# nv-tlabs/InfiniCube

Hardware: AMD Instinct MI355X
Metric: denoise steps/sec, 93-frame 480p Wan2.1 buffer-conditioned DiT loop (higher is better)
Workload: dtype bf16

## Files before the change

infinicube_amd/csrc/attention.hip:

```cpp
#include "icv_common.h"


int icv_attn1_dispatch(const void* q, int64_t ldq, const void* k, int64_t ldk, const void* v, int64_t ldv, void* o,
                       int64_t ldo, int64_t Sq, int64_t Skv, int64_t heads, float scale, void* stream);
int icv_attn2_dispatch(const void* q, int64_t ldq, const void* k, int64_t ldk, const void* v, int64_t ldv,
                       void* o, int64_t ldo, float* acc, int64_t ldacc, float* ml, int state_in,
                       int state_out, int64_t Sq, int64_t Skv, int64_t heads, float scale, int var,
                       hipStream_t st);

int icv_attn3_dispatch(const void* q, int64_t ldq, const void* k, int64_t ldk, const void* v, int64_t ldv,
                       void* o, int64_t ldo, float* acc, int64_t ldacc, float* ml, int state_in,
                       int state_out, int64_t Sq, int64_t Skv, int64_t heads, float scale, int var,
                       hipStream_t st);

int icv_attn9_dispatch(const void* q, int64_t ldq, const void* k, int64_t ldk, const void* v, int64_t ldv,
                       void* o, int64_t ldo, float* acc, int64_t ldacc, float* ml, int state_in,
                       int state_out, int64_t Sq, int64_t Skv, int64_t heads, float scale, int var,
                       hipStream_t st);
int icv_attn7p_single(const void* q, int64_t ldq, const void* k, int64_t ldk, const void* v, int64_t ldv, void* o, int64_t ldo, float* acc,
                      int64_t ldacc, float* ml, int state_in, int state_out, int64_t Sq, int64_t Skv, int64_t heads, float scale, hipStream_t st);
int icv_attn7q_single(const void* q, int64_t ldq, const void* k, int64_t ldk, const void* v, int64_t ldv, void* o, int64_t ldo, float* acc,
                      int64_t ldacc, float* ml, int state_in, int state_out, int64_t Sq, int64_t Skv, int64_t heads, float scale, int variant,
                      hipStream_t st);
int icv_attn7_dispatch(const void* q, int64_t ldq, const void* k, int64_t ldk, const void* v, int64_t ldv,
                       void* o, int64_t ldo, float* acc, int64_t ldacc, float* ml, int state_in,
                       int state_out, int64_t Sq, int64_t Skv, int64_t heads, float scale, int var,
                       hipStream_t st);
int icv_attn6_dispatch(const void* q, int64_t ldq, const void* k, int64_t ldk, const void* v, int64_t ldv,
                       void* o, int64_t ldo, float* acc, int64_t ldacc, float* ml, int state_in,
                       int state_out, int64_t Sq, int64_t Skv, int64_t heads, float scale, int var,
                       hipStream_t st);
int icv_attn5_dispatch(const void* q, int64_t ldq, const void* k, int64_t ldk, const void* v, int64_t ldv,
                       void* o, int64_t ldo, float* acc, int64_t ldacc, float* ml, int state_in,
                       int state_out, int64_t Sq, int64_t Skv, int64_t heads, float scale, int var,
                       hipStream_t st);
int icv_attn4_dispatch(const void* q, int64_t ldq, const void* k, int64_t ldk, const void* v, int64_t ldv,
                       void* o, int64_t ldo, float* acc, int64_t ldacc, float* ml, int state_in,
                       int state_out, int64_t Sq, int64_t Skv, int64_t heads, float scale, int var,
                       hipStream_t st);

constexpr int ATTN_KERNEL_DEFAULT = 7;
constexpr int ATTN7_VARIANT_DEFAULT = 132;
constexpr int ATTN7Q_DEFAULT = 0;
static int attn_route(const void* q, int64_t ldq, const void* k, int64_t ldk, const void* v, int64_t ldv, void* o,
                      int64_t ldo, float* acc, int64_t ldacc, float* ml, int state_in, int state_out, int64_t Sq,
                      int64_t Skv, int64_t heads, float scale, hipStream_t st) {
#define ATT_ARGS q, ldq, k, ldk, v, ldv, o, ldo, acc, ldacc, ml, state_in, state_out, Sq, Skv, heads, scale
  switch (icv_get_option_int("attn_kernel", ATTN_KERNEL_DEFAULT)) {
    case 7: {
      const int var7 = icv_get_option_int("attn7_variant", -1);
      int short_max = icv_get_option_int("attn7_short", -1);
      if (short_max < 0) short_max = 1024;
      if (var7 < 0 && Skv > short_max && !icv_get_option_int("attn7_plain", 0) && !icv_get_option_int("attn7_ablate", 0) && state_out != 2) {
#ifdef ICV_EXPERIMENTS
        const int q7 = icv_get_option_int("attn7q", ATTN7Q_DEFAULT);
        if (q7 > 0) {
          const int rc = icv_attn7q_single(ATT_ARGS, q7, st);
          if (rc >= 0) return rc;
        }
#endif
        return icv_attn7p_single(ATT_ARGS, st);
      }
      return icv_attn7_dispatch(ATT_ARGS, var7 < 0 ? ATTN7_VARIANT_DEFAULT : var7, st);
    }
#ifdef ICV_EXPERIMENTS
    case 9: return icv_attn9_dispatch(ATT_ARGS, icv_get_option_int("attn9_variant", 0), st);
    case 6: return icv_attn6_dispatch(ATT_ARGS, icv_get_option_int("attn6_variant", 5), st);
    case 5: return icv_attn5_dispatch(ATT_ARGS, 0, st);
    case 4: return icv_attn4_dispatch(ATT_ARGS, icv_get_option_int("attn4_variant", 4), st);
    case 3: return icv_attn3_dispatch(ATT_ARGS, icv_get_option_int("attn3_variant", 0), st);
#else
    case 9: case 6: case 5: case 4: case 3:
      icv_set_error("attn_kernel 3..6 and 9 are experiments: rebuild libicvideo with ICV_EXPERIMENTS=1");
      return 1;
#endif
    default: return icv_attn2_dispatch(ATT_ARGS, icv_get_option_int("attn2_variant", 12), st);
  }
#undef ATT_ARGS
}

extern "C" int icv_attention_fwd_chunk(const void* q, int64_t ldq, const void* k, int64_t ldk,
                                       const void* v, int64_t ldv, void* o, int64_t ldo, float* acc,
                                       int64_t ldacc, float* ml, int64_t Sq, int64_t Skv,
                                       int64_t heads, float scale, int first, int last, void* stream) {
  ICV_REQUIRE(q && k && v, "icv_attention_fwd_chunk: null pointer");
  ICV_REQUIRE(Sq > 0 && Skv > 0 && heads > 0, "icv_attention_fwd_chunk: empty problem");
  ICV_REQUIRE(ldq % 8 == 0 && ldk % 8 == 0 && ldv % 8 == 0, "icv_attention_fwd_chunk: leading dims must keep 16-byte row alignment");
  ICV_REQUIRE((first && last) || (acc && ml && ldacc % 4 == 0), "icv_attention_fwd_chunk: carried state buffers required unless first && last");
  ICV_REQUIRE(!last || (o && ldo % 4 == 0), "icv_attention_fwd_chunk: output required for the last chunk");
  return attn_route(q, ldq, k, ldk, v, ldv, o, ldo, acc, ldacc, ml, first ? 0 : 1, last ? 0 : 1, Sq, Skv, heads, scale, (hipStream_t)stream);
}

extern "C" int icv_attention_fwd(const void* q, int64_t ldq, const void* k, int64_t ldk,
                                 const void* v, int64_t ldv, void* o, int64_t ldo, int64_t Sq,
                                 int64_t Skv, int64_t heads, float scale, void* stream) {
  ICV_REQUIRE(q && k && v && o, "icv_attention_fwd: null pointer");
  ICV_REQUIRE(Sq > 0 && Skv > 0 && heads > 0, "icv_attention_fwd: empty problem (Sq=%lld Skv=%lld heads=%lld)", (long long)Sq, (long long)Skv, (long long)heads);
  ICV_REQUIRE(ldq % 8 == 0 && ldk % 8 == 0 && ldv % 8 == 0 && ldo % 4 == 0, "icv_attention_fwd: leading dims must keep 16-byte row alignment");
  if (icv_get_option_int("attn_kernel", ATTN_KERNEL_DEFAULT) != 1)
    return attn_route(q, ldq, k, ldk, v, ldv, o, ldo, nullptr, 0, nullptr, 0, 0, Sq, Skv, heads, scale, (hipStream_t)stream);
#ifdef ICV_EXPERIMENTS
  return icv_attn1_dispatch(q, ldq, k, ldk, v, ldv, o, ldo, Sq, Skv, heads, scale, stream);
#else
  icv_set_error("attn_kernel 1 is an experiment: rebuild libicvideo with ICV_EXPERIMENTS=1");
  return 1;
#endif
}

extern "C" int icv_attention_fwd_add(const void* q, int64_t ldq, const void* k, int64_t ldk,
                                     const void* v, int64_t ldv, void* o, int64_t ldo, int64_t Sq,
                                     int64_t Skv, int64_t heads, float scale, void* stream) {
  ICV_REQUIRE(q && k && v && o, "icv_attention_fwd_add: null pointer");
  ICV_REQUIRE(Sq > 0 && Skv > 0 && heads > 0, "icv_attention_fwd_add: empty problem (Sq=%lld Skv=%lld heads=%lld)", (long long)Sq, (long long)Skv, (long long)heads);
  ICV_REQUIRE(ldq % 8 == 0 && ldk % 8 == 0 && ldv % 8 == 0 && ldo % 4 == 0, "icv_attention_fwd_add: leading dims must keep 16-byte row alignment");
  return attn_route(q, ldq, k, ldk, v, ldv, o, ldo, nullptr, 0, nullptr, 0, 2, Sq, Skv, heads, scale, (hipStream_t)stream);
}

constexpr int ATTN_MFMA_DEFAULT = 16;
constexpr int ATTN_MFMA_SHORT_DEFAULT = 16;
int icv_attn_mfma(bool short_kv) {
  const int v = icv_get_option_int("attn_mfma", -1);
  if (v < 0) return short_kv ? ATTN_MFMA_SHORT_DEFAULT : ATTN_MFMA_DEFAULT;
  if (v == 16 || v == 32) return v;
  icv_set_error("attn_mfma = %d: the MFMA shape is 16 (16x16x32) or 32 (32x32x16); negative = the default", v);
  return -1;
}

constexpr int ATTN_TILE16_LEAN_DEFAULT = 1;
constexpr int ATTN_TILE16_LEAN_SHORT_DEFAULT = 1;
int icv_attn_tile16_lean(bool short_kv) {
  const int v = icv_get_option_int("attn_tile16_lean", -1);
  if (v < 0) return short_kv ? ATTN_TILE16_LEAN_SHORT_DEFAULT : ATTN_TILE16_LEAN_DEFAULT;
  if (v == 0 || v == 1) return v;
  icv_set_error("attn_tile16_lean = %d: 1 = the lean body of the 16x16x32 tile, 0 = the first body; negative = the default", v);
  return -1;
}

namespace {
unsigned long long* g_trace = nullptr;
int g_trace_cap = 0;
}
unsigned long long* icv_attention_trace_buffer(int* capacity) {
  *capacity = g_trace_cap;
  return g_trace;
}
extern "C" int icv_attention_trace(void* buf, int64_t capacity) {
  ICV_REQUIRE(capacity >= 0 && capacity < (1LL << 31), "icv_attention_trace: bad capacity");
  g_trace = (unsigned long long*)buf;
  g_trace_cap = buf ? (int)capacity : 0;
  return 0;
}
```

infinicube_amd/csrc/attn7p.hip:

```cpp
#include <type_traits>
#include "attn_common.h"

namespace att7p {

using attc::D;
using attc::NEG_BIG;
using attc::lds_read_tr16;
constexpr int KVB = 64;
constexpr int TILE_BYTES = KVB * D * 2;
constexpr int STAGE_BYTES = 2 * TILE_BYTES;
constexpr int NST = 4, NW = 8, NI = 16 / NW, QB = NW * 32;
constexpr int LDS_BYTES = NST * STAGE_BYTES + 64;
constexpr int MAX_PIECES = ICV_ATTN_MAX_PIECES;

struct Piece {
  const bf16_t* k;
  const bf16_t* v;
  int rows;
  int flag;
  unsigned value;
  int pad;
};

struct Params {
  attc::Params a;
  const unsigned* flags;
  unsigned* err;
  unsigned long long timeout_ticks;
  unsigned long long* ptrace;
  int n_pieces;
  Piece piece[MAX_PIECES];
  int fw_frames, fw_frame_rows, fw_window, fw_sink;
};

__device__ __forceinline__ void dma16(const void* gsrc, unsigned lds_dst) {
  unsigned keep;
  asm volatile(
      "s_mov_b32 %0, m0\n\t"
      "s_mov_b32 m0, %2\n\t"
      "s_nop 0\n\t"
      "global_load_lds_dwordx4 %1, off\n\t"
      "s_mov_b32 m0, %0"
      : "=&s"(keep)
      : "v"(gsrc), "s"(lds_dst)
      : "memory");
}

__device__ __forceinline__ void dma16s(const void* base, unsigned off, unsigned lds_dst) {
  unsigned keep;
  asm volatile(
      "s_mov_b32 %0, m0\n\t"
      "s_mov_b32 m0, %3\n\t"
      "s_nop 0\n\t"
      "global_load_lds_dwordx4 %1, %2\n\t"
      "s_mov_b32 m0, %0"
      : "=&s"(keep)
      : "v"(off), "s"(base), "s"(lds_dst)
      : "memory");
}

__device__ __forceinline__ unsigned load_flag_async(const unsigned* f) {
  unsigned v;
  asm volatile("global_load_dword %0, %1, off sc0 sc1" : "=v"(v) : "v"(f) : "memory");
  return v;
}

template <bool UNIT, bool FW, int MF, bool LEAN = false>
__global__ __launch_bounds__(NW * 64) __attribute__((amdgpu_waves_per_eu(2))) void attn7p_kernel(Params pp) {
  static_assert(MF == 16 || MF == 32, "MF: 16 (16x16x32 MFMAs) or 32 (32x32x16)");
  static_assert(MF == 16 || !LEAN, "the lean body is a body of the MF = 16 tile");
  const attc::Params& p = pp.a;
  const float p_lim = __builtin_amdgcn_exp2f(p.thr);
  extern __shared__ __attribute__((aligned(16))) char smem[];
  volatile unsigned* verdict = reinterpret_cast<volatile unsigned*>(smem + NST * STAGE_BYTES);
  const int tid = threadIdx.x;
  const int lane = tid & 63;
  const int wave = __builtin_amdgcn_readfirstlane(tid >> 6);
  const int hi = lane >> 5;
  const int l31 = lane & 31;

  int head, qb;
  attc::work_item(p, head, qb);
  int64_t q0 = (int64_t)qb * QB + wave * 32;
  int64_t q_end = 0;
  int fw_np = 1, fw_a0 = 0, fw_b0 = 0, fw_a1 = 0, fw_b1 = 0;
  if constexpr (FW) {
    const int T = pp.fw_frames, F = pp.fw_frame_rows, W = pp.fw_window, sink = pp.fw_sink;
    const int bpf = (F + QB - 1) / QB;
    const int f = qb / bpf;
    q0 = (int64_t)f * F + (qb - f * bpf) * QB + wave * 32;
    q_end = (int64_t)(f + 1) * F;
    const int lo = f - W > 0 ? f - W : 0;
    const int hi = f + W + 1 < T ? f + W + 1 : T;
    if (sink == 0) {
      fw_a0 = lo; fw_b0 = hi;
    } else if (lo <= sink) {
      fw_a0 = 0; fw_b0 = hi > sink ? hi : sink;
    } else {
      fw_np = 2;
      fw_a0 = 0; fw_b0 = sink;
      fw_a1 = lo; fw_b1 = hi;
    }
  }
  const unsigned long long t_start = p.trace ? __builtin_amdgcn_s_memrealtime() : 0ull;
  const bf16_t* qh = p.q + (int64_t)head * D;
  int64_t qr_c = q0 + l31;
  if constexpr (FW) qr_c = qr_c < q_end ? qr_c : q_end - 1;
  else qr_c = qr_c < p.Sq ? qr_c : p.Sq - 1;

  f32x16 ot[4];
  float m_run = NEG_BIG, l_run = 0.f;
  attc::Tile16 s16;
  int64_t qr16[2] = {0, 0};
  if constexpr (MF == 16) {
    const int64_t q_lim = FW ? q_end : p.Sq;
#pragma unroll
    for (int qb = 0; qb < 2; ++qb) {
      const int64_t r = q0 + qb * 16 + (lane & 15);
      qr16[qb] = r < q_lim ? r : q_lim - 1;
    }
    attc::tile16_init<UNIT>(p, qr16, head, lane >> 4, s16);
  } else {
    attc::load_state(p, qr_c, head, hi, ot, m_run, l_run);
  }
  float m_base = m_run < -1.0e29f ? 0.f : m_run;
  f32x16 cinit;
  const f32x16 zero16 = {0.f, 0.f, 0.f, 0.f, 0.f, 0.f, 0.f, 0.f, 0.f, 0.f, 0.f, 0.f, 0.f, 0.f, 0.f, 0.f};
#pragma unroll
  for (int r = 0; r < 16; ++r) cinit[r] = UNIT ? -m_base : 0.f;

  bf16x8 qf[8];
  if constexpr (MF == 16) attc::tile16_load_q(p, qr16, head, lane >> 4, s16);
  else {
    const bf16_t* qp = qh + qr_c * p.ldq + hi * 8;
#pragma unroll
    for (int ds = 0; ds < 8; ++ds) qf[ds] = *reinterpret_cast<const bf16x8*>(qp + ds * 16);
  }
  __builtin_amdgcn_s_waitcnt(0x0F70);

  const int pc = lane & 15;
  const unsigned lds_base = (unsigned)(uintptr_t)((__attribute__((address_space(3))) char*)smem);
  int dkey[NI], kcol[NI], vcol[NI];
  unsigned ko[NI], vo[NI];
#pragma unroll
  for (int j = 0; j < NI; ++j) {
    dkey[j] = (wave * NI + j) * 4 + (lane >> 4);
    kcol[j] = (pc ^ (dkey[j] & 15)) * 8;
    vcol[j] = MF == 16 ? attc::tile16_vcol(pc, dkey[j]) : (pc ^ ((dkey[j] & 3) << 2)) * 8;
    ko[j] = (unsigned)(((int64_t)dkey[j] * p.ldk + kcol[j]) * 2);
    vo[j] = (unsigned)(((int64_t)dkey[j] * p.ldv + vcol[j]) * 2);
  }

  const bf16_t* kh_d = nullptr;
  const bf16_t* vh_d = nullptr;
  int skv_d = 0, nt_d = 0;
#define P_ROWS(J_) (FW ? ((J_) ? fw_b1 - fw_a1 : fw_b0 - fw_a0) * pp.fw_frame_rows : __builtin_amdgcn_readfirstlane(pp.piece[FW ? 0 : (J_)].rows))
#define P_SET_DMA_PIECE(J_)                                              \
  {                                                                      \
    if constexpr (FW) {                                                  \
      const int64_t r0_ = (int64_t)((J_) ? fw_a1 : fw_a0) * pp.fw_frame_rows; \
      kh_d = p.k + r0_ * p.ldk + (int64_t)head * D;                      \
      vh_d = p.v + r0_ * p.ldv + (int64_t)head * D;                      \
      skv_d = P_ROWS(J_);                                                \
    } else {                                                             \
      const Piece& pc_ = pp.piece[(J_)];                                 \
      kh_d = pc_.k + (int64_t)head * D;                                  \
      vh_d = pc_.v + (int64_t)head * D;                                  \
      skv_d = __builtin_amdgcn_readfirstlane(pc_.rows);                  \
    }                                                                    \
    nt_d = (skv_d + KVB - 1) / KVB;                                      \
  }
#define P_DMA_TILE(T_, STG_)                                                                         \
  {                                                                                                  \
    const int tt_ = (T_) < nt_d ? (T_) : nt_d - 1;                                                   \
    const unsigned l0_ = lds_base + (unsigned)(((STG_) & (NST - 1)) * STAGE_BYTES + (wave * NI) * 1024); \
    if ((tt_ + 1) * KVB <= skv_d) {                                                                  \
      const bf16_t* kt_ = kh_d + (int64_t)tt_ * KVB * p.ldk;                                         \
      const bf16_t* vt_ = vh_d + (int64_t)tt_ * KVB * p.ldv;                                         \
      _Pragma("unroll") for (int j_ = 0; j_ < NI; ++j_) dma16s(kt_, ko[j_], l0_ + j_ * 1024);        \
      _Pragma("unroll") for (int j_ = 0; j_ < NI; ++j_) dma16s(vt_, vo[j_], l0_ + TILE_BYTES + j_ * 1024); \
    } else {                                                                                         \
      _Pragma("unroll") for (int j_ = 0; j_ < NI; ++j_) {                                            \
        int64_t r_ = (int64_t)tt_ * KVB + dkey[j_];                                                  \
        r_ = r_ < skv_d ? r_ : skv_d - 1;                                                            \
        dma16(kh_d + r_ * p.ldk + kcol[j_], l0_ + j_ * 1024);                                        \
        dma16(vh_d + r_ * p.ldv + vcol[j_], l0_ + TILE_BYTES + j_ * 1024);                           \
      }                                                                                              \
    }                                                                                                \
  }
#define P_BARRIER()                                           \
  do {                                                        \
    asm volatile("s_waitcnt lgkmcnt(0)" ::: "memory");        \
    __builtin_amdgcn_s_barrier();                             \
    asm volatile("" ::: "memory");                            \
    __builtin_amdgcn_sched_barrier(0);                        \
  } while (0)
#define P_WAIT_PIECE(J_)                                                                                          \
  if constexpr (!FW) {                                                                                            \
    const int fi_ = __builtin_amdgcn_readfirstlane(pp.piece[(J_)].flag);                                          \
    if (fi_ >= 0) {                                                                                               \
      if (tid == 0) {                                                                                             \
        const unsigned want_ = pp.piece[(J_)].value;                                                              \
        const unsigned long long t0_ = __builtin_amdgcn_s_memrealtime();                                          \
        while ((int)(__hip_atomic_load(pp.flags + fi_, __ATOMIC_RELAXED, __HIP_MEMORY_SCOPE_SYSTEM) - want_) < 0) { \
          __builtin_amdgcn_s_sleep(16);                                                                           \
              \
          if (pp.err && __hip_atomic_load(pp.err, __ATOMIC_RELAXED, __HIP_MEMORY_SCOPE_AGENT) != 0u) break;       \
          if (pp.timeout_ticks && __builtin_amdgcn_s_memrealtime() - t0_ > pp.timeout_ticks) {                    \
            if (pp.err) atomicCAS(pp.err, 0u, 0x80000000u | (unsigned)(J_));                                      \
            break;                                                                                                \
          }                                                                                                       \
        }                                                                                                         \
      }                                                                                                           \
      P_BARRIER();                                                                                                \
    }                                                                                                             \
  }

  const int k_row_off = l31 * 256;
  const int k_sw = l31 & 15;
  const int g = lane >> 4, t16 = lane & 15;
  const int v_key_lo = 4 * hi + (t16 >> 2);
  const int v_byte_lo = (g & 1) * 32 + (t16 & 3) * 8;
  const int v_sw = (t16 >> 2) << 6;

  attc::Tile16Addr la16;
  int la16_step = 2 * STAGE_BYTES;
  if constexpr (LEAN) {
    attc::tile16_lean_addr(lds_base, lane, la16);
    attc::tile16_lean_lim<UNIT>(s16, p_lim, la16);
  }
  auto tile = [&](const auto par, const int stg, const int key0, const int skv) __attribute__((always_inline)) {
    if constexpr (LEAN) {
      attc::tile16<UNIT, false, true, true, true, decltype(par)::value>(p, p_lim, nullptr, nullptr, key0, skv, lane, s16, &la16);
      return;
    }
    const char* ks = smem + (stg & (NST - 1)) * STAGE_BYTES;
    const char* vs = ks + TILE_BYTES;
    if constexpr (MF == 16) {
      attc::tile16<UNIT, false, true, true>(p, p_lim, ks, vs, key0, skv, lane, s16);
      return;
    }
    f32x16 st[2];
    const bool no_ref = UNIT && m_run < -1.0e29f;
#pragma unroll
    for (int ds = 0; ds < 8; ++ds)
#pragma unroll
      for (int kb = 0; kb < 2; ++kb) {
        const int c = ds * 2 + hi;
        const bf16x8 kf = *reinterpret_cast<const bf16x8*>(ks + kb * 8192 + k_row_off + ((c ^ k_sw) << 4));
        st[kb] = __builtin_amdgcn_mfma_f32_32x32x16_bf16(kf, qf[ds], ds == 0 ? (UNIT ? cinit : zero16) : st[kb], 0, 0, 0);
      }
    if (key0 + KVB > skv) {
#pragma unroll
      for (int kb = 0; kb < 2; ++kb)
#pragma unroll
        for (int r = 0; r < 16; ++r) {
          const int key = key0 + kb * 32 + (r & 3) + 8 * (r >> 2) + 4 * hi;
          if (key >= skv) st[kb][r] = NEG_BIG;
        }
    }
    float mb = -m_run * p.sc;
    float psum = 0.f;
    __builtin_amdgcn_s_setprio(1);
#pragma unroll
    for (int kb = 0; kb < 2; ++kb) {
      bf16x8 pf[2];
      float ps = 0.f;
#pragma unroll
      for (int r = 0; r < 16; ++r) {
        const float pv = UNIT ? __builtin_amdgcn_exp2f(st[kb][r]) : __builtin_amdgcn_exp2f(fmaf(st[kb][r], p.sc, mb));
        ps += pv;
        pf[r >> 3][r & 7] = (__bf16)pv;
      }
      if (__any(!(ps <= p_lim) || no_ref)) {
        float mloc = st[kb][0];
#pragma unroll
        for (int r = 1; r < 16; ++r) mloc = fmaxf(mloc, st[kb][r]);
        mloc = fmaxf(mloc, __shfl_xor(mloc, 32, 64));
        if (UNIT) mloc += m_base;
        const float m_new = fmaxf(m_run, mloc);
        const float alpha = __builtin_amdgcn_exp2f((m_run - m_new) * p.sc);
        m_run = m_new;
        l_run = (l_run + psum) * alpha;
        psum = 0.f;
#pragma unroll
        for (int i = 0; i < 4; ++i)
#pragma unroll
          for (int r = 0; r < 16; ++r) ot[i][r] *= alpha;
        mb = -m_run * p.sc;
        if (UNIT) {
          const float dm = m_new - m_base;
          m_base = m_new;
#pragma unroll
          for (int j = 0; j < 2; ++j)
            if (j >= kb) {
#pragma unroll
              for (int r = 0; r < 16; ++r) st[j][r] -= dm;
            }
#pragma unroll
          for (int r = 0; r < 16; ++r) cinit[r] = -m_new;
        }
        ps = 0.f;
#pragma unroll
        for (int r = 0; r < 16; ++r) {
          const float pv = UNIT ? __builtin_amdgcn_exp2f(st[kb][r]) : __builtin_amdgcn_exp2f(fmaf(st[kb][r], p.sc, mb));
          ps += pv;
          pf[r >> 3][r & 7] = (__bf16)pv;
        }
      }
      psum += ps;
#pragma unroll
      for (int hf = 0; hf < 2; ++hf) {
        const int kk = kb * 2 + hf;
#pragma unroll
        for (int d0 = 0; d0 < 4; ++d0) {
          const int key_l = kk * 16 + v_key_lo;
          const int byte = (d0 * 64 + v_byte_lo) ^ v_sw;
          const bf16x4 va = lds_read_tr16(vs + key_l * 256 + byte);
          const bf16x4 vb = lds_read_tr16(vs + (key_l + 8) * 256 + byte);
          bf16x8 vf;
          vf[0] = va[0]; vf[1] = va[1]; vf[2] = va[2]; vf[3] = va[3];
          vf[4] = vb[0]; vf[5] = vb[1]; vf[6] = vb[2]; vf[7] = vb[3];
          ot[d0] = __builtin_amdgcn_mfma_f32_32x32x16_bf16(vf, pf[hf], ot[d0], 0, 0, 0);
        }
      }
    }
    __builtin_amdgcn_s_setprio(0);
    l_run += psum;
  };

  const int np = FW ? fw_np : __builtin_amdgcn_readfirstlane(pp.n_pieces);
  if constexpr (MF == 16) __builtin_assume(np >= 1);
  unsigned gt = 0;
  unsigned iv = 0;
  P_WAIT_PIECE(0);
  P_SET_DMA_PIECE(0);
  P_DMA_TILE(0, gt);
  P_DMA_TILE(1, gt + 1);
  asm volatile("s_waitcnt vmcnt(0)" ::: "memory");
  P_BARRIER();
  for (int pj = 0; pj < np; ++pj) {
    const int skv = P_ROWS(pj);
    const int nt = (skv + KVB - 1) / KVB;
    if constexpr (MF == 16) __builtin_assume(nt >= 1);
    const unsigned g_next = gt + (unsigned)((nt + 1) & ~1);
    const bool has_next = pj + 1 < np;
    const int nflag = has_next && !FW ? __builtin_amdgcn_readfirstlane(pp.piece[has_next ? pj + 1 : pj].flag) : -1;
    const unsigned nvalue = has_next && !FW ? pp.piece[has_next ? pj + 1 : pj].value : 0u;
    bool next_ready = has_next && nflag < 0;
    bool next_issued = false;
    if (!FW && pp.ptrace && tid == 0) pp.ptrace[(size_t)blockIdx.x * np + pj] = __builtin_amdgcn_s_memrealtime();
    for (int t = 0; t < nt; t += 2) {
      const bool last_iv = t + 2 >= nt;
      if (!last_iv) {
        P_DMA_TILE(t + 2, gt + t + 2);
        P_DMA_TILE(t + 3, gt + t + 3);
      } else if (has_next && next_ready) {
        P_SET_DMA_PIECE(pj + 1);
        P_DMA_TILE(0, g_next);
        P_DMA_TILE(1, g_next + 1);
        next_issued = true;
      }
      const bool poll = has_next && !next_ready;
      unsigned fv = 0;
      if (poll && wave == 0) fv = load_flag_async(pp.flags + nflag);
      tile(std::integral_constant<int, 0>{}, (int)(gt + t), t * KVB, skv);
      if (t + 1 < nt) tile(std::integral_constant<int, 1>{}, (int)(gt + t + 1), (t + 1) * KVB, skv);
      if constexpr (LEAN) {
        attc::tile16_lean_advance(la16, la16_step);
        la16_step = -la16_step;
      }
      asm volatile("s_waitcnt vmcnt(0)" ::: "memory");
      if (poll && tid == 0) verdict[iv & 1] = (int)(fv - nvalue) >= 0 ? 1u : 0u;
      P_BARRIER();
      if (poll) next_ready = __builtin_amdgcn_readfirstlane(verdict[iv & 1]) != 0;
      ++iv;
    }
    if (!has_next) break;
    if (!next_issued) {
      if (!next_ready) P_WAIT_PIECE(pj + 1);
      P_SET_DMA_PIECE(pj + 1);
      P_DMA_TILE(0, g_next);
      P_DMA_TILE(1, g_next + 1);
      asm volatile("s_waitcnt vmcnt(0)" ::: "memory");
      P_BARRIER();
    }
    gt = g_next;
  }
  asm volatile("s_waitcnt vmcnt(0)" ::: "memory");

  if constexpr (MF == 16) {
    int64_t qr[2];
    int t16 = lane & 15;
    asm volatile("" : "+v"(t16));
#pragma unroll
    for (int qb = 0; qb < 2; ++qb) {
      const int64_t r = q0 + qb * 16 + t16;
      qr[qb] = !FW || r < q_end ? r : p.Sq;
    }
    attc::store_result(p, qr, head, lane >> 4, s16.ot, s16.m_run, s16.l_run);
  } else {
    attc::store_result(p, !FW || q0 + l31 < q_end ? q0 + l31 : p.Sq, head, hi, ot, m_run, l_run);
  }
  if (p.trace && tid == 0 && (int)blockIdx.x < p.trace_cap) {
    unsigned hwid, xcc;
    asm volatile("s_getreg_b32 %0, hwreg(HW_REG_HW_ID)" : "=s"(hwid));
    asm volatile("s_getreg_b32 %0, hwreg(HW_REG_XCC_ID)" : "=s"(xcc));
    unsigned long long* t = p.trace + (size_t)blockIdx.x * 4;
    t[0] = t_start; t[1] = __builtin_amdgcn_s_memrealtime(); t[2] = hwid; t[3] = xcc;
  }
#undef P_ROWS
#undef P_SET_DMA_PIECE
#undef P_DMA_TILE
#undef P_BARRIER
#undef P_WAIT_PIECE
}

template <bool UNIT, bool FW, int MF, bool LEAN = false>
int launch_mf(const Params& pp, hipStream_t st) {
  static icv_dev_flags attr_set = {};
  if (int rc = icv_ensure_dynamic_lds((const void*)attn7p_kernel<UNIT, FW, MF, LEAN>, LDS_BYTES, &attr_set, "attn7p")) return rc;
  const int64_t nwg = (int64_t)pp.a.heads * pp.a.nqb;
  hipLaunchKernelGGL((attn7p_kernel<UNIT, FW, MF, LEAN>), dim3((unsigned)nwg), dim3(NW * 64), LDS_BYTES, st, pp);
  return icv_check_launch(FW ? "icv_attention_fwd_framewin" : "icv_attention_fwd_pieces");
}

template <bool UNIT, bool FW = false>
int launch(const Params& pp, hipStream_t st) {
  const int mf = icv_attn_mfma(false);
  if (mf < 0) return 1;
  if (mf != 16) return launch_mf<UNIT, FW, 32>(pp, st);
  const int lean = icv_attn_tile16_lean(false);
  if (lean < 0) return 1;
  return lean ? launch_mf<UNIT, FW, 16, true>(pp, st) : launch_mf<UNIT, FW, 16>(pp, st);
}

}

extern "C" int icv_attention_fwd_pieces(const void* q, int64_t ldq, const icv_kv_piece* pieces, int64_t n_pieces, int64_t ldk, int64_t ldv,
                                        void* o, int64_t ldo, int64_t Sq, int64_t heads, float scale, const uint32_t* flags, uint32_t* err,
                                        int64_t timeout_us, void* trace, void* stream) {
  ICV_REQUIRE(q && pieces && o, "icv_attention_fwd_pieces: null pointer");
  ICV_REQUIRE(Sq > 0 && heads > 0 && n_pieces > 0, "icv_attention_fwd_pieces: empty problem (Sq=%lld heads=%lld pieces=%lld)", (long long)Sq,
              (long long)heads, (long long)n_pieces);
  ICV_REQUIRE(ldq % 8 == 0 && ldk % 8 == 0 && ldv % 8 == 0 && ldo % 4 == 0, "icv_attention_fwd_pieces: leading dims must keep 16-byte row alignment");
  att7p::Params pp;
  int64_t total = 0;
  int n = 0;
  for (int64_t i = 0; i < n_pieces; ++i) {
    const icv_kv_piece& s = pieces[i];
    ICV_REQUIRE(s.rows >= 0 && s.rows < (1LL << 31) / 64, "icv_attention_fwd_pieces: piece %lld has %lld rows", (long long)i, (long long)s.rows);
    if (s.rows == 0) continue;
    ICV_REQUIRE(n < att7p::MAX_PIECES, "icv_attention_fwd_pieces: more than %d non-empty pieces", att7p::MAX_PIECES);
    ICV_REQUIRE(s.k && s.v, "icv_attention_fwd_pieces: piece %lld has a null pointer", (long long)i);
    ICV_REQUIRE(s.flag < 0 || flags, "icv_attention_fwd_pieces: piece %lld waits for flag %d but no flag array was given", (long long)i, s.flag);
    ICV_REQUIRE(64 * ldk * 2 < (1LL << 32) && 64 * ldv * 2 < (1LL << 32), "icv_attention_fwd_pieces: row stride too large");
    att7p::Piece& d = pp.piece[n++];
    d.k = (const bf16_t*)s.k; d.v = (const bf16_t*)s.v; d.rows = (int)s.rows; d.flag = s.flag; d.value = s.value; d.pad = 0;
    total += s.rows;
  }
  ICV_REQUIRE(n > 0, "icv_attention_fwd_pieces: every piece is empty");
  attc::fill_params(pp.a, q, ldq, nullptr, ldk, nullptr, ldv, o, ldo, nullptr, 0, nullptr, 0, 0, Sq, total, heads, scale, 256);
  pp.a.trace = icv_attention_trace_buffer(&pp.a.trace_cap);
  pp.flags = flags;
  pp.err = err;
  pp.timeout_ticks = timeout_us > 0 ? (unsigned long long)timeout_us * 100ull : 0ull;
  pp.ptrace = (unsigned long long*)trace;
  pp.n_pieces = n;
  hipStream_t st = (hipStream_t)stream;
  return (pp.a.sc == 1.0f && icv_get_option_int("attn_unit_scale", 1)) ? att7p::launch<true>(pp, st) : att7p::launch<false>(pp, st);
}

int icv_attn7p_single(const void* q, int64_t ldq, const void* k, int64_t ldk, const void* v, int64_t ldv, void* o, int64_t ldo, float* acc,
                      int64_t ldacc, float* ml, int state_in, int state_out, int64_t Sq, int64_t Skv, int64_t heads, float scale, hipStream_t st) {
  ICV_REQUIRE(Skv > 0 && Skv < (1LL << 31) / 64 && 64 * ldk * 2 < (1LL << 32) && 64 * ldv * 2 < (1LL << 32), "icv_attention: key axis / row stride too large");
  att7p::Params pp;
  attc::fill_params(pp.a, q, ldq, nullptr, ldk, nullptr, ldv, o, ldo, acc, ldacc, ml, state_in, state_out, Sq, Skv, heads, scale, 256);
  pp.a.trace = icv_attention_trace_buffer(&pp.a.trace_cap);
  pp.flags = nullptr; pp.err = nullptr; pp.timeout_ticks = 0; pp.ptrace = nullptr;
  pp.n_pieces = 1;
  att7p::Piece& d = pp.piece[0];
  d.k = (const bf16_t*)k; d.v = (const bf16_t*)v; d.rows = (int)Skv; d.flag = -1; d.value = 0; d.pad = 0;
  return (pp.a.sc == 1.0f && icv_get_option_int("attn_unit_scale", 1)) ? att7p::launch<true>(pp, st) : att7p::launch<false>(pp, st);
}

extern "C" int icv_attention_fwd_framewin(const void* q, int64_t ldq, const void* k, int64_t ldk, const void* v, int64_t ldv, void* o, int64_t ldo,
                                          int64_t frames, int64_t frame_rows, int64_t heads, int64_t window, int64_t sink, float scale, void* stream) {
  ICV_REQUIRE(q && k && v && o, "icv_attention_fwd_framewin: null pointer");
  ICV_REQUIRE(frames > 0 && frame_rows > 0 && heads > 0, "icv_attention_fwd_framewin: empty problem (frames=%lld frame_rows=%lld heads=%lld)",
              (long long)frames, (long long)frame_rows, (long long)heads);
  ICV_REQUIRE(window >= 0 && sink >= 0, "icv_attention_fwd_framewin: window (%lld) and sink (%lld) must be >= 0", (long long)window, (long long)sink);
  ICV_REQUIRE(sink <= frames, "icv_attention_fwd_framewin: sink (%lld) exceeds the %lld frames", (long long)sink, (long long)frames);
  ICV_REQUIRE(ldq % 8 == 0 && ldk % 8 == 0 && ldv % 8 == 0 && ldo % 4 == 0, "icv_attention_fwd_framewin: leading dims must keep 16-byte row alignment");
  ICV_REQUIRE(frames < (1LL << 31) / 64 && frame_rows < (1LL << 31) / 64 && frames * frame_rows < (1LL << 31) / 64,
              "icv_attention_fwd_framewin: %lld frames of %lld rows: key axis too large", (long long)frames, (long long)frame_rows);
  ICV_REQUIRE(64 * ldk * 2 < (1LL << 32) && 64 * ldv * 2 < (1LL << 32), "icv_attention_fwd_framewin: row stride too large");
  const int64_t nqb = frames * ((frame_rows + att7p::QB - 1) / att7p::QB);
  ICV_REQUIRE(heads * nqb < (1LL << 31), "icv_attention_fwd_framewin: %lld work-groups", (long long)(heads * nqb));
  att7p::Params pp;
  attc::fill_params(pp.a, q, ldq, k, ldk, v, ldv, o, ldo, nullptr, 0, nullptr, 0, 0, frames * frame_rows, frames * frame_rows, heads, scale, 256);
  pp.a.nqb = (int)nqb;
  pp.a.trace = icv_attention_trace_buffer(&pp.a.trace_cap);
  pp.flags = nullptr; pp.err = nullptr; pp.timeout_ticks = 0; pp.ptrace = nullptr;
  pp.n_pieces = 0;
  pp.fw_frames = (int)frames;
  pp.fw_frame_rows = (int)frame_rows;
  pp.fw_window = (int)(window < frames ? window : frames);
  pp.fw_sink = (int)sink;
  hipStream_t st = (hipStream_t)stream;
  return (pp.a.sc == 1.0f && icv_get_option_int("attn_unit_scale", 1)) ? att7p::launch<true, true>(pp, st) : att7p::launch<false, true>(pp, st);
}

namespace {
__global__ void flag_write_kernel(uint32_t* flag, uint32_t value, unsigned long long delay_ticks) {
  if (delay_ticks) {
    const unsigned long long t0 = __builtin_amdgcn_s_memrealtime();
    while (__builtin_amdgcn_s_memrealtime() - t0 < delay_ticks) __builtin_amdgcn_s_sleep(32);
  }
  __hip_atomic_store(flag, value, __ATOMIC_RELEASE, __HIP_MEMORY_SCOPE_SYSTEM);
}
}

extern "C" int icv_flag_write(uint32_t* flags, int64_t index, uint32_t value, int64_t delay_us, void* stream) {
  ICV_REQUIRE(flags && index >= 0, "icv_flag_write: bad argument");
  ICV_REQUIRE(delay_us >= 0 && delay_us <= 10000000, "icv_flag_write: delay_us out of range");
  hipLaunchKernelGGL(flag_write_kernel, dim3(1), dim3(1), 0, (hipStream_t)stream, flags + index, value, (unsigned long long)delay_us * 100ull);
  return icv_check_launch("icv_flag_write");
}
```

infinicube_amd/csrc/attn_common.h:

```cpp
#pragma once
#include "icv_common.h"

unsigned long long* icv_attention_trace_buffer(int* capacity);
int icv_attn_mfma(bool short_kv);
int icv_attn_tile16_lean(bool short_kv);

namespace attc {

constexpr int D = 128;
constexpr float NEG_BIG = -1.0e30f;

struct Params {
  const bf16_t* q; int64_t ldq;
  const bf16_t* k; int64_t ldk;
  const bf16_t* v; int64_t ldv;
  bf16_t* o; int64_t ldo;
  float* acc; int64_t ldacc;
  float* ml;
  int64_t Sq, Skv;
  int heads, nqb;
  int state_in, state_out;
  float sc;
  float thr;
  int ablate;
  unsigned long long* trace;
  int trace_cap;
};


inline void fill_params(Params& p, const void* q, int64_t ldq, const void* k, int64_t ldk, const void* v,
                        int64_t ldv, void* o, int64_t ldo, float* acc, int64_t ldacc, float* ml, int state_in,
                        int state_out, int64_t Sq, int64_t Skv, int64_t heads, float scale, int rows_per_block) {
  p.q = (const bf16_t*)q; p.ldq = ldq; p.k = (const bf16_t*)k; p.ldk = ldk;
  p.v = (const bf16_t*)v; p.ldv = ldv; p.o = (bf16_t*)o; p.ldo = ldo;
  p.acc = acc; p.ldacc = ldacc; p.ml = ml; p.state_in = state_in; p.state_out = state_out;
  p.Sq = Sq; p.Skv = Skv; p.heads = (int)heads;
  p.nqb = (int)((Sq + rows_per_block - 1) / rows_per_block);
  p.sc = scale * 1.4426950408889634f;
  if (fabsf(p.sc - 1.0f) < 1e-6f) p.sc = 1.0f;
  p.thr = (float)icv_get_option_int("attn_defer_max_log2", 8);
  p.ablate = 0;
  p.trace = nullptr;
  p.trace_cap = 0;
}

typedef __attribute__((address_space(3))) s16x4 lds_s16x4;

__device__ __forceinline__ bf16x4 lds_read_tr16(const char* p) {
  s16x4 r = __builtin_amdgcn_ds_read_tr16_b64_v4i16((lds_s16x4*)(p));
  return __builtin_bit_cast(bf16x4, r);
}

__device__ __forceinline__ void work_item(const Params& p, int& head, int& qb) {
  const int nwg = p.heads * p.nqb;
  const int bid = blockIdx.x;
  const int xcd = bid & 7, local = bid >> 3;
  const int qn = nwg >> 3, r = nwg & 7;
  const int wg = (xcd < r ? xcd * (qn + 1) : r * (qn + 1) + (xcd - r) * qn) + local;
  head = wg / p.nqb;
  qb = wg - head * p.nqb;
}

__device__ __forceinline__ void load_state(const Params& p, int64_t qr_c, int head, int hi, f32x16 (&ot)[4],
                                           float& m_run, float& l_run) {
  if (p.state_in) {
    const float* ap = p.acc + qr_c * p.ldacc + (int64_t)head * D + 4 * hi;
#pragma unroll
    for (int d0 = 0; d0 < 4; ++d0)
#pragma unroll
      for (int rr = 0; rr < 4; ++rr) {
        const float4 a = *reinterpret_cast<const float4*>(ap + d0 * 32 + rr * 8);
        ot[d0][rr * 4 + 0] = a.x; ot[d0][rr * 4 + 1] = a.y; ot[d0][rr * 4 + 2] = a.z; ot[d0][rr * 4 + 3] = a.w;
      }
    const float2 mlv = *reinterpret_cast<const float2*>(p.ml + (qr_c * p.heads + head) * 2);
    m_run = mlv.x;
    l_run = hi == 0 ? mlv.y : 0.f;
  } else {
#pragma unroll
    for (int i = 0; i < 4; ++i)
#pragma unroll
      for (int r = 0; r < 16; ++r) ot[i][r] = 0.f;
    m_run = NEG_BIG;
    l_run = 0.f;
  }
}

__device__ __forceinline__ void store_result(const Params& p, int64_t qr, int head, int hi, const f32x16 (&ot)[4],
                                             float m_run, float l_run) {
  const float l_tot = l_run + __shfl_xor(l_run, 32, 64);
  if (qr >= p.Sq) return;
  if (p.state_out == 1) {
    float* ap = p.acc + qr * p.ldacc + (int64_t)head * D + 4 * hi;
#pragma unroll
    for (int d0 = 0; d0 < 4; ++d0)
#pragma unroll
      for (int rr = 0; rr < 4; ++rr)
        *reinterpret_cast<float4*>(ap + d0 * 32 + rr * 8) =
            make_float4(ot[d0][rr * 4 + 0], ot[d0][rr * 4 + 1], ot[d0][rr * 4 + 2], ot[d0][rr * 4 + 3]);
    if (hi == 0) *reinterpret_cast<float2*>(p.ml + (qr * p.heads + head) * 2) = make_float2(m_run, l_tot);
  } else {
    const float inv = 1.0f / l_tot;
    bf16_t* op = p.o + qr * p.ldo + (int64_t)head * D + 4 * hi;
#pragma unroll
    for (int d0 = 0; d0 < 4; ++d0)
#pragma unroll
      for (int rr = 0; rr < 4; ++rr) {
        float a = ot[d0][rr * 4 + 0] * inv, b = ot[d0][rr * 4 + 1] * inv;
        float c = ot[d0][rr * 4 + 2] * inv, d = ot[d0][rr * 4 + 3] * inv;
        if (p.state_out == 2) {
          const uint2 prev = *reinterpret_cast<const uint2*>(op + d0 * 32 + rr * 8);
          a += __uint_as_float(prev.x << 16); b += __uint_as_float(prev.x & 0xFFFF0000u);
          c += __uint_as_float(prev.y << 16); d += __uint_as_float(prev.y & 0xFFFF0000u);
        }
        *reinterpret_cast<uint2*>(op + d0 * 32 + rr * 8) = make_uint2(pack_bf16x2(a, b), pack_bf16x2(c, d));
      }
  }
}

struct Tile16 {
  f32x4 ot[8][2];
  float m_run[2], l_run[2], m_base[2];
  f32x4 cinit[2];
  bf16x8 qf[2][4];
};

__device__ __forceinline__ void load_state(const Params& p, const int64_t (&qr_c)[2], int head, int g, f32x4 (&ot)[8][2],
                                           float (&m_run)[2], float (&l_run)[2]) {
#pragma unroll
  for (int qb = 0; qb < 2; ++qb) {
    if (p.state_in) {
      const float* ap = p.acc + qr_c[qb] * p.ldacc + (int64_t)head * D + 4 * g;
#pragma unroll
      for (int db = 0; db < 8; ++db) {
        const float4 a = *reinterpret_cast<const float4*>(ap + db * 16);
        ot[db][qb][0] = a.x; ot[db][qb][1] = a.y; ot[db][qb][2] = a.z; ot[db][qb][3] = a.w;
      }
      const float2 mlv = *reinterpret_cast<const float2*>(p.ml + (qr_c[qb] * p.heads + head) * 2);
      m_run[qb] = mlv.x;
      l_run[qb] = g == 0 ? mlv.y : 0.f;
    } else {
#pragma unroll
      for (int db = 0; db < 8; ++db)
#pragma unroll
        for (int r = 0; r < 4; ++r) ot[db][qb][r] = 0.f;
      m_run[qb] = NEG_BIG;
      l_run[qb] = 0.f;
    }
  }
}

__device__ __forceinline__ void store_result(const Params& p, const int64_t (&qr)[2], int head, int g, const f32x4 (&ot)[8][2],
                                             const float (&m_run)[2], const float (&l_run)[2]) {
  float l_tot[2];
#pragma unroll
  for (int qb = 0; qb < 2; ++qb) {
    const float l2 = l_run[qb] + __shfl_xor(l_run[qb], 16, 64);
    l_tot[qb] = l2 + __shfl_xor(l2, 32, 64);
  }
#pragma unroll
  for (int qb = 0; qb < 2; ++qb) {
    if (qr[qb] >= p.Sq) continue;
    if (p.state_out == 1) {
      float* ap = p.acc + qr[qb] * p.ldacc + (int64_t)head * D + 4 * g;
#pragma unroll
      for (int db = 0; db < 8; ++db)
        *reinterpret_cast<float4*>(ap + db * 16) = make_float4(ot[db][qb][0], ot[db][qb][1], ot[db][qb][2], ot[db][qb][3]);
      if (g == 0) *reinterpret_cast<float2*>(p.ml + (qr[qb] * p.heads + head) * 2) = make_float2(m_run[qb], l_tot[qb]);
    } else {
      const float inv = 1.0f / l_tot[qb];
      bf16_t* op = p.o + qr[qb] * p.ldo + (int64_t)head * D + 4 * g;
#pragma unroll
      for (int db = 0; db < 8; ++db) {
        float a = ot[db][qb][0] * inv, b = ot[db][qb][1] * inv;
        float c = ot[db][qb][2] * inv, d = ot[db][qb][3] * inv;
        if (p.state_out == 2) {
          const uint2 prev = *reinterpret_cast<const uint2*>(op + db * 16);
          a += __uint_as_float(prev.x << 16); b += __uint_as_float(prev.x & 0xFFFF0000u);
          c += __uint_as_float(prev.y << 16); d += __uint_as_float(prev.y & 0xFFFF0000u);
        }
        *reinterpret_cast<uint2*>(op + db * 16) = make_uint2(pack_bf16x2(a, b), pack_bf16x2(c, d));
      }
    }
  }
}

__device__ __forceinline__ void tile16_load_q(const Params& p, const int64_t (&qr_c)[2], int head, int g, Tile16& s) {
  const bf16_t* qh = p.q + (int64_t)head * D + g * 8;
#pragma unroll
  for (int qb = 0; qb < 2; ++qb)
#pragma unroll
    for (int ks = 0; ks < 4; ++ks) s.qf[qb][ks] = *reinterpret_cast<const bf16x8*>(qh + qr_c[qb] * p.ldq + ks * 32);
}

template <bool UNIT>
__device__ __forceinline__ void tile16_init(const Params& p, const int64_t (&qr_c)[2], int head, int g, Tile16& s) {
  load_state(p, qr_c, head, g, s.ot, s.m_run, s.l_run);
#pragma unroll
  for (int qb = 0; qb < 2; ++qb) {
    s.m_base[qb] = s.m_run[qb] < -1.0e29f ? 0.f : s.m_run[qb];
#pragma unroll
    for (int r = 0; r < 4; ++r) s.cinit[qb][r] = UNIT ? -s.m_base[qb] : 0.f;
  }
}

__device__ __forceinline__ int tile16_vcol(int pc, int key) { return (pc ^ ((key & 7) << 1)) * 8; }

typedef __attribute__((address_space(3))) bf16x8 lds_bf16x8;
struct Tile16Addr {
  unsigned k[4], v[8];
  float lim[2];
};
template <bool UNIT>
__device__ __forceinline__ void tile16_lean_lim(const Tile16& s, const float p_lim, Tile16Addr& a) {
#pragma unroll
  for (int qb = 0; qb < 2; ++qb) a.lim[qb] = UNIT && s.m_run[qb] < -1.0e29f ? -1.0f : p_lim;
}
__device__ __forceinline__ void tile16_lean_addr(const unsigned lds_base, const int lane, Tile16Addr& a) {
  const int g = lane >> 4, t = lane & 15;
  const int v_row_off = (4 * g + (t >> 2)) * 256;
  const int v_sw = (4 * (g & 1) + (t >> 2)) << 5;
  const int v_byte_lo = (t & 3) * 8;
#pragma unroll
  for (int ks = 0; ks < 4; ++ks) a.k[ks] = lds_base + t * 256 + (((ks * 4 + g) ^ t) << 4);
#pragma unroll
  for (int db = 0; db < 8; ++db) a.v[db] = lds_base + 16384 + v_row_off + ((db * 32 + v_byte_lo) ^ v_sw);
}
__device__ __forceinline__ void tile16_lean_advance(Tile16Addr& a, const int bytes) {
#pragma unroll
  for (int ks = 0; ks < 4; ++ks) a.k[ks] += (unsigned)bytes;
#pragma unroll
  for (int db = 0; db < 8; ++db) a.v[db] += (unsigned)bytes;
}

__device__ __forceinline__ float t16_add_opaque(const float a, const float b, const float one) { return __builtin_fmaf(b, one, a); }

template <bool UNIT, bool KPREFETCH, bool DSMAJOR, bool SETPRIO, bool LEAN = false, int STG = 0>
__device__ __forceinline__ void tile16(const Params& p, const float p_lim, const char* ks, const char* vs, const int64_t key0,
                                       const int64_t skv, const int lane, Tile16& s, Tile16Addr* la = nullptr) {
  static_assert(STG == 0 || (LEAN && STG == 1), "STG: the tile's place in a step of two stages (lean body only)");
  static_assert(STG * 32768 + 8192 + 4096 < 65536, "the ds_read offset: field holds 16 bits");
  const int g = lane >> 4, t = lane & 15;
  const f32x4 zero4 = {0.f, 0.f, 0.f, 0.f};
  const int k_row_off = t * 256;
  const int v_row_off = (4 * g + (t >> 2)) * 256;
  const int v_sw = (4 * (g & 1) + (t >> 2)) << 5;
  const int v_byte_lo = (t & 3) * 8;
  f32x4 st[4][2];
  const bool no_ref = UNIT && !LEAN && (s.m_run[0] < -1.0e29f || s.m_run[1] < -1.0e29f);
#define T16_KADDR(KB_, KS_) (ks + (KB_) * 4096 + k_row_off + ((((KS_) * 4 + g) ^ t) << 4))
#define T16_KLOAD(DST_, KB_, KS_)                                                                                   \
  do {                                                                                                              \
    if constexpr (LEAN) DST_ = *(const lds_bf16x8*)(la->k[KS_] + (unsigned)(STG * 32768 + (KB_) * 4096));           \
    else DST_ = *reinterpret_cast<const bf16x8*>(T16_KADDR(KB_, KS_));                                              \
  } while (0)
#define T16_QK(KB_, KS_, KF_)                                                                                       \
  _Pragma("unroll") for (int qb = 0; qb < 2; ++qb) st[KB_][qb] = __builtin_amdgcn_mfma_f32_16x16x32_bf16(           \
      KF_, s.qf[qb][KS_], (KS_) == 0 ? (UNIT ? s.cinit[qb] : zero4) : st[KB_][qb], 0, 0, 0)
  if (KPREFETCH) {
    bf16x8 kf[4][4];
#pragma unroll
    for (int kb = 0; kb < 4; ++kb)
#pragma unroll
      for (int kq = 0; kq < 4; ++kq) T16_KLOAD(kf[kb][kq], kb, kq);
    __builtin_amdgcn_sched_barrier(0);
    if (SETPRIO) __builtin_amdgcn_s_setprio(1);
#pragma unroll
    for (int kq = 0; kq < 4; ++kq)
#pragma unroll
      for (int kb = 0; kb < 4; ++kb) { T16_QK(kb, kq, kf[kb][kq]); }
    if (SETPRIO) __builtin_amdgcn_s_setprio(0);
  } else if (DSMAJOR) {
    constexpr int KD = 3;
    bf16x8 kf[16];
#pragma unroll
    for (int i = 0; i < KD; ++i) T16_KLOAD(kf[i], i & 3, i >> 2);
#pragma unroll
    for (int i = 0; i < 16; ++i) {
      if (i + KD < 16) T16_KLOAD(kf[i + KD], (i + KD) & 3, (i + KD) >> 2);
      T16_QK(i & 3, i >> 2, kf[i]);
    }
    __builtin_amdgcn_sched_group_barrier(0x100, KD, 0);
#pragma unroll
    for (int i = 0; i < 16; ++i) {
      if (i + KD < 16) __builtin_amdgcn_sched_group_barrier(0x100, 1, 0);
      __builtin_amdgcn_sched_group_barrier(0x008, 2, 0);
    }
  } else {
    if (SETPRIO) __builtin_amdgcn_s_setprio(1);
#pragma unroll
    for (int kb = 0; kb < 4; ++kb)
#pragma unroll
      for (int kq = 0; kq < 4; ++kq) {
        bf16x8 kf;
        T16_KLOAD(kf, kb, kq);
        T16_QK(kb, kq, kf);
      }
    if (SETPRIO) __builtin_amdgcn_s_setprio(0);
  }
#undef T16_KADDR
#undef T16_KLOAD
#undef T16_QK
  if (key0 + 64 > skv) {
#pragma unroll
    for (int kb = 0; kb < 4; ++kb)
#pragma unroll
      for (int r = 0; r < 4; ++r) {
        const int64_t key = key0 + kb * 16 + 4 * g + r;
        if (key >= skv) { st[kb][0][r] = NEG_BIG; st[kb][1][r] = NEG_BIG; }
      }
  }
  float one = 1.0f;
  if (LEAN) asm("" : "+s"(one));
  float mb[2] = {-s.m_run[0] * p.sc, -s.m_run[1] * p.sc};
  float psum[2] = {0.f, 0.f};
  if (SETPRIO) __builtin_amdgcn_s_setprio(1);
#pragma unroll
  for (int kk = 0; kk < 2; ++kk) {
    bf16x8 pf[2];
    float ps[2];
#define T16_EXP()                                                                                                   \
  _Pragma("unroll") for (int qb = 0; qb < 2; ++qb) {                                                                \
    ps[qb] = 0.f;                                                                                                   \
    _Pragma("unroll") for (int j = 0; j < 8; ++j) {                                                                 \
      const float sv = st[2 * kk + (j >> 2)][qb][j & 3];                                                            \
      const float pv = UNIT ? __builtin_amdgcn_exp2f(sv) : __builtin_amdgcn_exp2f(fmaf(sv, p.sc, mb[qb]));          \
      if (LEAN && j == 0) ps[qb] = pv;                                                         \
      else if (LEAN && qb == 1) ps[qb] = t16_add_opaque(ps[qb], pv, one);                                           \
      else ps[qb] += pv;                                                                                            \
      pf[qb][j] = (__bf16)pv;                                                                                       \
    }                                                                                                               \
  }
    T16_EXP();
    if (__any(LEAN && UNIT ? !(ps[0] <= la->lim[0]) || !(ps[1] <= la->lim[1]) : !(ps[0] <= p_lim) || !(ps[1] <= p_lim) || no_ref)) {
#pragma unroll
      for (int qb = 0; qb < 2; ++qb) {
        float mloc = st[2 * kk][qb][0];
#pragma unroll
        for (int j = 1; j < 8; ++j) mloc = fmaxf(mloc, st[2 * kk + (j >> 2)][qb][j & 3]);
        mloc = fmaxf(mloc, __shfl_xor(mloc, 16, 64));
        mloc = fmaxf(mloc, __shfl_xor(mloc, 32, 64));
        if (UNIT) mloc += s.m_base[qb];
        const float m_new = fmaxf(s.m_run[qb], mloc);
        const float alpha = __builtin_amdgcn_exp2f((s.m_run[qb] - m_new) * p.sc);
        s.m_run[qb] = m_new;
        if (LEAN && UNIT && kk == 1) la->lim[qb] = m_new < -1.0e29f ? -1.0f : p_lim;
        s.l_run[qb] = (s.l_run[qb] + psum[qb]) * alpha;
        psum[qb] = 0.f;
#pragma unroll
        for (int db = 0; db < 8; ++db)
#pragma unroll
          for (int r = 0; r < 4; ++r) s.ot[db][qb][r] *= alpha;
        mb[qb] = -m_new * p.sc;
        if (UNIT) {
          const float dm = m_new - s.m_base[qb];
          s.m_base[qb] = m_new;
#pragma unroll
          for (int kb = 0; kb < 4; ++kb)
            if (kb >= 2 * kk) {
#pragma unroll
              for (int r = 0; r < 4; ++r) st[kb][qb][r] -= dm;
            }
#pragma unroll
          for (int r = 0; r < 4; ++r) s.cinit[qb][r] = -m_new;
        }
      }
      T16_EXP();
    }
#undef T16_EXP
    if (LEAN) {
      psum[0] = kk == 0 ? ps[0] : psum[0] + ps[0];
      psum[1] = kk == 0 ? ps[1] : t16_add_opaque(psum[1], ps[1], one);
    } else {
      psum[0] += ps[0];
      psum[1] += ps[1];
    }
    constexpr int VD = 2;
    bf16x4 va[8], vb[8];
#define T16_VREAD(DB_)                                                                                  \
  {                                                                                                     \
    if constexpr (LEAN) {                                                                               \
      const unsigned va_a = la->v[DB_] + (unsigned)(STG * 32768 + kk * 8192);                           \
      va[DB_] = __builtin_bit_cast(bf16x4, __builtin_amdgcn_ds_read_tr16_b64_v4i16((lds_s16x4*)(va_a))); \
      vb[DB_] = __builtin_bit_cast(bf16x4, __builtin_amdgcn_ds_read_tr16_b64_v4i16((lds_s16x4*)(va_a + 4096u))); \
    } else {                                                                                            \
      const char* va_p = vs + kk * 8192 + v_row_off + (((DB_) * 32 + v_byte_lo) ^ v_sw);                 \
      va[DB_] = lds_read_tr16(va_p);                                                                    \
      vb[DB_] = lds_read_tr16(va_p + 4096);  \
    }                                                                                                   \
  }
#pragma unroll
    for (int db = 0; db < VD; ++db) T16_VREAD(db);
#pragma unroll
    for (int db = 0; db < 8; ++db) {
      if (db + VD < 8) T16_VREAD(db + VD);
      bf16x8 vf;
      vf[0] = va[db][0]; vf[1] = va[db][1]; vf[2] = va[db][2]; vf[3] = va[db][3];
      vf[4] = vb[db][0]; vf[5] = vb[db][1]; vf[6] = vb[db][2]; vf[7] = vb[db][3];
#pragma unroll
      for (int qb = 0; qb < 2; ++qb) s.ot[db][qb] = __builtin_amdgcn_mfma_f32_16x16x32_bf16(vf, pf[qb], s.ot[db][qb], 0, 0, 0);
    }
#undef T16_VREAD
    __builtin_amdgcn_sched_group_barrier(0x100, 2 * VD, 0);
#pragma unroll
    for (int db = 0; db < 8; ++db) {
      if (db + VD < 8) __builtin_amdgcn_sched_group_barrier(0x100, 2, 0);
      __builtin_amdgcn_sched_group_barrier(0x008, 2, 0);
    }
  }
  if (SETPRIO) __builtin_amdgcn_s_setprio(0);
  s.l_run[0] += psum[0];
  if (LEAN) s.l_run[1] = t16_add_opaque(s.l_run[1], psum[1], one);
  else s.l_run[1] += psum[1];
}

}
```

Baseline: 0.3017.

## Add slim steady-state key loop to attn7p pieces kernel

Adds a specialized steady-state loop for the pieces attention kernel (lean 16x16x32 body) that issues K/V tile DMAs through one inline-asm block with immediate offsets. It advances the tile pointers and the LDS stage address incrementally and drops the per-tile bounds, flag and piece checks. The general loop still handles the tail tiles. It is on by default when the leading dims are at least D, and it adds a new template variant plus fragile asm that sets m0 and assumes NI == 2.

```diff
diff --git a/infinicube_amd/csrc/attention.hip b/infinicube_amd/csrc/attention.hip
--- a/infinicube_amd/csrc/attention.hip
+++ b/infinicube_amd/csrc/attention.hip
@@ -136,6 +136,15 @@
   return -1;
 }
 
+constexpr int ATTN7P_SLIM_DEFAULT = 1;
+int icv_attn7p_slim() {
+  const int v = icv_get_option_int("attn7p_slim", -1);
+  if (v < 0) return ATTN7P_SLIM_DEFAULT;
+  if (v == 0 || v == 1) return v;
+  icv_set_error("attn7p_slim = %d: 1 = the slim key loop of attn7p, 0 = the one loop; negative = the default", v);
+  return -1;
+}
+
 namespace {
 unsigned long long* g_trace = nullptr;
 int g_trace_cap = 0;
diff --git a/infinicube_amd/csrc/attn7p.hip b/infinicube_amd/csrc/attn7p.hip
--- a/infinicube_amd/csrc/attn7p.hip
+++ b/infinicube_amd/csrc/attn7p.hip
@@ -59,16 +59,36 @@
       : "memory");
 }
 
+#pragma clang diagnostic push
+#pragma clang diagnostic ignored "-Winline-asm"
+__device__ __forceinline__ void dma_tile_slim(const void* kt, const void* vt, unsigned ko0, unsigned ko1, unsigned vo0, unsigned vo1,
+                                              unsigned lds_dst) {
+  asm volatile(
+      "s_mov_b32 m0, %6\n\t"
+      "s_nop 0\n\t"
+      "global_load_lds_dwordx4 %0, %4\n\t"
+      "global_load_lds_dwordx4 %1, %4 offset:1024\n\t"
+      "s_add_u32 m0, %6, %7\n\t"
+      "s_nop 0\n\t"
+      "global_load_lds_dwordx4 %2, %5\n\t"
+      "global_load_lds_dwordx4 %3, %5 offset:1024"
+      :
+      : "v"(ko0), "v"(ko1), "v"(vo0), "v"(vo1), "s"(kt), "s"(vt), "s"(lds_dst), "i"(TILE_BYTES)
+      : "memory", "m0", "scc");
+}
+#pragma clang diagnostic pop
+
 __device__ __forceinline__ unsigned load_flag_async(const unsigned* f) {
   unsigned v;
   asm volatile("global_load_dword %0, %1, off sc0 sc1" : "=v"(v) : "v"(f) : "memory");
   return v;
 }
 
-template <bool UNIT, bool FW, int MF, bool LEAN = false>
+template <bool UNIT, bool FW, int MF, bool SLIM = false, bool LEAN = false>
 __global__ __launch_bounds__(NW * 64) __attribute__((amdgpu_waves_per_eu(2))) void attn7p_kernel(Params pp) {
   static_assert(MF == 16 || MF == 32, "MF: 16 (16x16x32 MFMAs) or 32 (32x32x16)");
   static_assert(MF == 16 || !LEAN, "the lean body is a body of the MF = 16 tile");
+  static_assert(LEAN || !SLIM, "the slim loop is a loop around the lean body");
   const attc::Params& p = pp.a;
   const float p_lim = __builtin_amdgcn_exp2f(p.thr);
   extern __shared__ __attribute__((aligned(16))) char smem[];
@@ -147,8 +167,8 @@
     dkey[j] = (wave * NI + j) * 4 + (lane >> 4);
     kcol[j] = (pc ^ (dkey[j] & 15)) * 8;
     vcol[j] = MF == 16 ? attc::tile16_vcol(pc, dkey[j]) : (pc ^ ((dkey[j] & 3) << 2)) * 8;
-    ko[j] = (unsigned)(((int64_t)dkey[j] * p.ldk + kcol[j]) * 2);
-    vo[j] = (unsigned)(((int64_t)dkey[j] * p.ldv + vcol[j]) * 2);
+    ko[j] = (unsigned)(((int64_t)dkey[j] * p.ldk + kcol[j]) * 2) - (SLIM ? j * 1024u : 0u);
+    vo[j] = (unsigned)(((int64_t)dkey[j] * p.ldv + vcol[j]) * 2) - (SLIM ? j * 1024u : 0u);
   }
 
   const bf16_t* kh_d = nullptr;
@@ -177,8 +197,8 @@
     if ((tt_ + 1) * KVB <= skv_d) {                                                                  \
       const bf16_t* kt_ = kh_d + (int64_t)tt_ * KVB * p.ldk;                                         \
       const bf16_t* vt_ = vh_d + (int64_t)tt_ * KVB * p.ldv;                                         \
-      _Pragma("unroll") for (int j_ = 0; j_ < NI; ++j_) dma16s(kt_, ko[j_], l0_ + j_ * 1024);        \
-      _Pragma("unroll") for (int j_ = 0; j_ < NI; ++j_) dma16s(vt_, vo[j_], l0_ + TILE_BYTES + j_ * 1024); \
+      _Pragma("unroll") for (int j_ = 0; j_ < NI; ++j_) dma16s(kt_ + (SLIM ? j_ * 512 : 0), ko[j_], l0_ + j_ * 1024); \
+      _Pragma("unroll") for (int j_ = 0; j_ < NI; ++j_) dma16s(vt_ + (SLIM ? j_ * 512 : 0), vo[j_], l0_ + TILE_BYTES + j_ * 1024); \
     } else {                                                                                         \
       _Pragma("unroll") for (int j_ = 0; j_ < NI; ++j_) {                                            \
         int64_t r_ = (int64_t)tt_ * KVB + dkey[j_];                                                  \
@@ -350,7 +370,37 @@
     bool next_ready = has_next && nflag < 0;
     bool next_issued = false;
     if (!FW && pp.ptrace && tid == 0) pp.ptrace[(size_t)blockIdx.x * np + pj] = __builtin_amdgcn_s_memrealtime();
-    for (int t = 0; t < nt; t += 2) {
+    int t_steady = 0;
+    if constexpr (SLIM) {
+      int t = 0;
+      const int t_last = (skv >> 6) - 6;
+      if (t_last >= 0) {
+        const int64_t kstep = (int64_t)KVB * p.ldk, vstep = (int64_t)KVB * p.ldv;
+        const bf16_t* kt_d = kh_d + 2 * kstep;
+        const bf16_t* vt_d = vh_d + 2 * vstep;
+        const unsigned l_w = lds_base + (unsigned)(wave * NI * 1024);
+        unsigned l0_d = l_w + (unsigned)(((gt + 2) & (NST - 1)) * STAGE_BYTES);
+        const unsigned l_sum = 2 * l_w + 2 * STAGE_BYTES;
+        int yes = 1;
+        asm volatile("" : "+s"(yes));
+        static_assert(NI == 2, "dma_tile_slim issues two K and two V pieces per wave");
+        for (; t <= t_last; t += 2) {
+          dma_tile_slim(kt_d, vt_d, ko[0], ko[1], vo[0], vo[1], l0_d);
+          dma_tile_slim(kt_d + kstep, vt_d + vstep, ko[0], ko[1], vo[0], vo[1], l0_d + STAGE_BYTES);
+          kt_d += 2 * kstep;
+          vt_d += 2 * vstep;
+          l0_d = l_sum - l0_d;
+          tile(std::integral_constant<int, 0>{}, 0, 0, KVB);
+          if (yes) tile(std::integral_constant<int, 1>{}, 0, 0, KVB);
+          attc::tile16_lean_advance(la16, la16_step);
+          la16_step = -la16_step;
+          asm volatile("s_waitcnt vmcnt(0)" ::: "memory");
+          P_BARRIER();
+        }
+        t_steady = t;
+      }
+    }
+    for (int t = SLIM ? t_steady : 0; t < nt; t += 2) {
       const bool last_iv = t + 2 >= nt;
       if (!last_iv) {
         P_DMA_TILE(t + 2, gt + t + 2);
@@ -416,12 +466,12 @@
 #undef P_WAIT_PIECE
 }
 
-template <bool UNIT, bool FW, int MF, bool LEAN = false>
+template <bool UNIT, bool FW, int MF, bool SLIM = false, bool LEAN = false>
 int launch_mf(const Params& pp, hipStream_t st) {
   static icv_dev_flags attr_set = {};
-  if (int rc = icv_ensure_dynamic_lds((const void*)attn7p_kernel<UNIT, FW, MF, LEAN>, LDS_BYTES, &attr_set, "attn7p")) return rc;
+  if (int rc = icv_ensure_dynamic_lds((const void*)attn7p_kernel<UNIT, FW, MF, SLIM, LEAN>, LDS_BYTES, &attr_set, "attn7p")) return rc;
   const int64_t nwg = (int64_t)pp.a.heads * pp.a.nqb;
-  hipLaunchKernelGGL((attn7p_kernel<UNIT, FW, MF, LEAN>), dim3((unsigned)nwg), dim3(NW * 64), LDS_BYTES, st, pp);
+  hipLaunchKernelGGL((attn7p_kernel<UNIT, FW, MF, SLIM, LEAN>), dim3((unsigned)nwg), dim3(NW * 64), LDS_BYTES, st, pp);
   return icv_check_launch(FW ? "icv_attention_fwd_framewin" : "icv_attention_fwd_pieces");
 }
 
@@ -432,7 +482,13 @@
   if (mf != 16) return launch_mf<UNIT, FW, 32>(pp, st);
   const int lean = icv_attn_tile16_lean(false);
   if (lean < 0) return 1;
-  return lean ? launch_mf<UNIT, FW, 16, true>(pp, st) : launch_mf<UNIT, FW, 16>(pp, st);
+  if (!lean) return launch_mf<UNIT, FW, 16>(pp, st);
+  if constexpr (!FW) {
+    const int slim = icv_attn7p_slim();
+    if (slim < 0) return 1;
+    if (slim && pp.a.ldk >= D && pp.a.ldv >= D) return launch_mf<UNIT, FW, 16, true, true>(pp, st);
+  }
+  return launch_mf<UNIT, FW, 16, false, true>(pp, st);
 }
 
 }
diff --git a/infinicube_amd/csrc/attn_common.h b/infinicube_amd/csrc/attn_common.h
--- a/infinicube_amd/csrc/attn_common.h
+++ b/infinicube_amd/csrc/attn_common.h
@@ -4,6 +4,7 @@
 unsigned long long* icv_attention_trace_buffer(int* capacity);
 int icv_attn_mfma(bool short_kv);
 int icv_attn_tile16_lean(bool short_kv);
+int icv_attn7p_slim();
 
 namespace attc {
 
```

After: 0.3072 (median of 6 runs). 1.8% higher.
